# SHI-Labs/SH-GAN

Measured on AMD Instinct MI355X. Metric: generator images/sec, higher is better.
Workload: dtype f32

## Files before the change

include/shgan_hip.h:

```cpp
#ifndef SHGAN_HIP_H
#define SHGAN_HIP_H
#include <stddef.h>
#include <stdint.h>
#ifdef __cplusplus
extern "C" {
#endif

#define SHG_OK 0
#define SHG_ERR_ARG (-1)
#define SHG_ERR_LAUNCH (-2)
#define SHG_ERR_UNSUPPORTED (-3)

int shg_abi_version(void);
const char* shg_last_error(void);
int shg_device_info(int dev, char* buf, int buflen);

int shg_upfirdn2d_out_size(int H, int W, int fh, int fw, int upx, int upy, int downx, int downy, int padx0, int padx1,
                           int pady0, int pady1, int* OH, int* OW);
int shg_upfirdn2d_f32(const float* x, const float* f, float* y, int N, int C, int H, int W, int fh, int fw, int upx, int upy,
                      int downx, int downy, int padx0, int padx1, int pady0, int pady1, int flip, float gain, void* stream);
int shg_upfirdn2d_strided(const void* x, const float* f, void* y, int dtype, int N, int C, int H, int W, const long* x_strides,
                          const long* y_strides, int fh, int fw, long f_stride_y, long f_stride_x, int upx, int upy, int downx, int downy,
                          int padx0, int padx1, int pady0, int pady1, int flip, float gain, void* stream);
int shg_upfirdn2d_epilogue_f32(const float* x, const float* f, float* y, int N, int C, int H, int W, int fh, int fw, int upx,
// ... 54 lines not shown
                             int act, float alpha, float act_gain, float clamp, const float* residual, void* stream);
int shg_conv_weight_prep_up_poly_f32(const float* w, const float* wscale, float* wu_a, float* wu_b, int O, int I, int OP, int flip,
                                     void* stream);
int shg_conv2d_up_poly_supported(int NB, int I, int O, int H, int W);
int shg_conv2d_up_poly_f32(const float* x, const float* wt, const float* wu_a, const float* wu_b, float* y, int NB, int I, int O,
                           int OP, int H, int W, const float* in_scale, void* stream);
size_t shg_conv2d_up_poly_workspace_bytes(int NB, int I, int O, int OP, int H, int W);
int shg_conv2d_up_poly_ws_f32(const float* x, const float* wt, const float* wu_a, const float* wu_b, float* y, int NB, int I, int O,
                              int OP, int H, int W, const float* in_scale, void* workspace, size_t ws_bytes, void* stream);
int shg_fir_down_planar_f32(const float* x, const float* f, float* y, int N, int C, int H, int W, int PP, int flip, float gain,
                            void* stream);
int shg_fir_pad2_sep_supported(int H, int W, int PP);
int shg_fir_pad2_sep_f32(const float* x, const float* taps_host, float* y, int N, int C, int H, int W, int PP, int flip, float gain,
                         void* stream);
int shg_fir_resample2_sep_supported(int H, int W, int up);
int shg_fir_resample2_sep_f32(const float* x, const float* taps_host, float* y, int N, int C, int H, int W, int up, int flip, float gain,
                              void* stream);
int shg_conv_weight_prep_down_poly_f32(const float* w, const float* wscale, float* wu_a, float* wu_b, int O, int I, int OP, int flip,
                                       void* stream);
int shg_conv2d_down_poly_supported(int NB, int I, int O, int OH, int OW);
int shg_conv2d_down_poly_f32(const float* xp, const float* wu_a, const float* wu_b, float* y, int NB, int I, int O, int OP, int OH,
                             int OW, int PP, const float* in_scale, const float* bias, int act, float alpha, float gain,
                             float clamp, const float* residual, void* stream);
int shg_conv1x1_thin_in_f32(const float* x, const float* w, const float* bias, float* y, int N, int I, int O, int HW, float wgain,
                            int act, float alpha, float gain, float clamp, void* stream);
int shg_torgb_f32(const float* x, const float* w, const float* styles, const float* bias, const float* base_up, const float* f,
                  float* y, int N, int I, int O, int H, int W, void* stream);

int shg_dense_f32(const float* x, const float* w, const float* b, float* y, int N, int K, int O, int ldx, int ldy, float wgain,
                  float bgain, int act, float alpha, float gain, float clamp, void* stream);
int shg_matmul_nn_f32(const float* a, const float* b, float* out, int N, int M, int K, int lda, int ldo, float scale, void* stream);
int shg_matmul_tn_f32(const float* a, const float* b, float* out, float* colsum, int N, int M, int K, int lda, int ldb, float scale,
                      float csum_scale, void* stream);
int shg_demod_weight_f32(const float* w, float* wn, float* wsq, float* sfac, int O, int I, int K, int prenorm, void* stream);
int shg_demod_weight_backward_f32(const float* wn, const float* sfac, const float* gwn, const float* gwsq, float* gw, int O, int I, int K,
                                  void* stream);
int shg_style_factors_f32(const float* s, const float* wsq, float* sn, float* d, float* aux, int N, int I, int O, int prenorm, void* stream);
int shg_style_factors_backward_f32(const float* sn, const float* d, const float* wsq, const float* aux, const float* gsn, const float* gd,
                                   float* gs, float* gwsq, float* partq, int N, int I, int O, int prenorm, void* stream);
int shg_normalize_2nd_moment_f32(const float* x, float* y, int N, int K, float eps, void* stream);
int shg_modconv_style_prep_f32(const float* styles, int ld, const float* wsq, float* s_out, float* dcoef, int N, int I, int O,
                               int OP, int demod, float pre_gain, void* stream);

typedef struct {
    const float* x1; const float* x2; const float* w; const float* b; float* y;
    int ld1, ld2, K1, K2, O, ldy;
// ... 78 lines not shown
```

sh-gan_amd/_lib.py:

```python
import ctypes
import os

import torch

_HERE = os.path.dirname(os.path.abspath(__file__))
LIB_PATH = os.path.join(_HERE, 'lib', 'libshgan_hip.so')
ABI_VERSION = 38

c_fp = ctypes.c_void_p
c_i = ctypes.c_int
c_f = ctypes.c_float
c_l = ctypes.c_long
c_pp = ctypes.POINTER(ctypes.c_void_p)



class DenseGroup(ctypes.Structure):
    _fields_ = [('x1', c_fp), ('x2', c_fp), ('w', c_fp), ('b', c_fp), ('y', c_fp),
                ('ld1', c_i), ('ld2', c_i), ('K1', c_i), ('K2', c_i), ('O', c_i), ('ldy', c_i),
                ('wgain', c_f), ('bgain', c_f)]


class StyleGroup(ctypes.Structure):
    _fields_ = [('styles', c_fp), ('wsq', c_fp), ('s_out', c_fp), ('dcoef', c_fp),
                ('ld', c_i), ('I', c_i), ('O', c_i), ('OP', c_i), ('demod', c_i), ('pre_gain', c_f)]


_SIGS = {
    'shg_abi_version': [],
    'shg_device_info': [c_i, ctypes.c_char_p, c_i],
# ... 47 lines not shown
    'shg_conv2d_wgrad_f32': [c_fp, c_fp, c_fp] + [c_i] * 11 + [c_fp, ctypes.c_size_t, c_fp],
    'shg_conv2d_wgrad_wino_supported': [c_i] * 8,
    'shg_conv2d_wgrad_wino_workspace_bytes': [c_i] * 5,
    'shg_conv2d_wgrad_wino_f32': [c_fp, c_fp, c_fp] + [c_i] * 5 + [c_fp, ctypes.c_size_t, c_fp],
    'shg_shu_spectral_f32': [c_fp] * 6 + [c_i] * 4 + [c_fp],
    'shg_shu_split_irfft2_f32': [c_fp, c_fp, c_pp, c_pp, ctypes.POINTER(c_l), c_i, c_i, c_i, c_i, c_fp],
    'shg_shu_split_adjoint_f32': [c_pp, ctypes.POINTER(c_l), c_pp, c_fp, c_i, c_i, c_fp],
    'shg_composite_u8': [c_fp, c_fp, c_fp, c_i, c_i, c_i, c_fp],
    'shg_assemble_input_f32': [c_fp, c_fp, c_fp, c_i, c_i, c_i, c_fp],
    'shg_assemble_input_u8': [c_fp, c_fp, c_fp, c_fp, c_i, c_i, c_i, c_fp],
    'shg_conv_weight_prep_up_poly_f32': [c_fp, c_fp, c_fp, c_fp, c_i, c_i, c_i, c_i, c_fp],
    'shg_conv2d_up_poly_supported': [c_i, c_i, c_i, c_i, c_i],
    'shg_conv2d_up_poly_f32': [c_fp, c_fp, c_fp, c_fp, c_fp, c_i, c_i, c_i, c_i, c_i, c_i, c_fp, c_fp],
    'shg_conv2d_up_poly_ws_f32': [c_fp, c_fp, c_fp, c_fp, c_fp] + [c_i] * 6 + [c_fp, c_fp, ctypes.c_size_t, c_fp],
    'shg_conv2d_up_poly_workspace_bytes': [c_i] * 6,
    'shg_fir_down_planar_f32': [c_fp, c_fp, c_fp, c_i, c_i, c_i, c_i, c_i, c_i, c_f, c_fp],
    'shg_fir_pad2_sep_supported': [c_i, c_i, c_i],
    'shg_fir_resample2_sep_supported': [c_i, c_i, c_i],
    'shg_fir_resample2_sep_f32': [c_fp, ctypes.POINTER(c_f), c_fp, c_i, c_i, c_i, c_i, c_i, c_i, c_f, c_fp],
    'shg_fir_pad2_sep_f32': [c_fp, ctypes.POINTER(c_f), c_fp, c_i, c_i, c_i, c_i, c_i, c_i, c_f, c_fp],
    'shg_conv_weight_prep_down_poly_f32': [c_fp, c_fp, c_fp, c_fp, c_i, c_i, c_i, c_i, c_fp],
    'shg_conv2d_down_poly_supported': [c_i, c_i, c_i, c_i, c_i],
    'shg_conv2d_down_poly_f32': [c_fp, c_fp, c_fp, c_fp, c_i, c_i, c_i, c_i, c_i, c_i, c_i, c_fp, c_fp, c_i, c_f, c_f, c_f, c_fp, c_fp],
    'shg_mask_raster_f32': [c_fp, c_fp, c_fp, c_fp, c_i, c_fp, c_fp, c_i, c_i, c_fp],
    'shg_fid_accumulate_f64': [c_fp, c_i, c_fp, c_fp, c_i, c_i, c_i, c_fp],
    'shg_image_metrics_scratch_bytes': [c_i] * 4,
    'shg_image_metrics': [c_fp, c_fp, c_f, c_f, c_fp, c_fp, c_f, c_f] + [c_i] * 6 + [c_fp, ctypes.c_size_t, c_fp, c_fp, c_fp],
    'shg_resize_bicubic_u8': [c_fp, c_l, c_fp, c_l, c_fp, c_i, c_i, c_i, c_i, c_i, c_fp],
    'shg_minibatch_std_f32': [c_fp, c_fp, c_fp, c_i, c_i, c_i, c_i, c_i, c_i, c_fp],
    'shg_conv2d_f16': [c_fp, c_fp, c_fp, c_fp] + [c_i] * 12 + [c_fp],
    'shg_conv2d_f16_needs_clear': [c_i] * 5,
    'shg_conv2d_f16_fused': [c_fp, c_fp, c_fp] + [c_i] * 12 + [c_fp, c_fp, c_fp, c_i, c_f, c_fp, c_i, c_f, c_f, c_f, c_fp, c_fp],
    'shg_conv2d_f16_packed_weight_elems': [c_i] * 3,
    'shg_conv2d_f16_pack_weight': [c_fp, c_fp, c_i, c_i, c_i, c_fp],
    'shg_conv2d_f16_pack_weight_oihw': [c_fp, c_fp, c_i, c_i, c_i, c_i, c_i, c_fp],
    'shg_conv2d_f16_set_routes': [c_i],
    'shg_conv2d_wgrad_f16_workspace_bytes': [c_i] * 6,
    'shg_conv2d_wgrad_f16': [c_fp, c_fp, c_fp] + [c_i] * 10 + [c_fp, ctypes.c_size_t, c_fp],
    'shg_upfirdn2d_f16': [c_fp, c_fp, c_fp] + [c_i] * 15 + [c_f, c_fp],
    'shg_relayout_f32_f16': [c_fp, c_fp, c_i, c_i, c_l, c_i, c_fp],
    'shg_bias_act_f16': [c_fp, c_fp, c_fp, c_l, c_i, c_i, c_f, c_f, c_f, c_fp],
    'shg_bias_act_backward_f16': [c_fp, c_fp, c_fp, c_l, c_i, c_f, c_f, c_f, c_fp],
    'shg_modtail_backward_f32_blocks': [c_l],
    'shg_modtail_backward_f32_cslices': [c_i, c_i, c_l],
    'shg_modtail_backward_f32': [c_fp] * 9 + [c_i, c_i, c_l, c_i, c_f, c_f, c_f, c_fp],
    'shg_modtail_f16': [c_fp, c_fp, c_fp, c_i, c_fp, c_fp, c_i, c_l, c_i, c_i, c_f, c_f, c_f, c_fp],
# ... 18 lines not shown
    if _lib is not None:
        return _lib
    if not os.path.exists(LIB_PATH):
        raise RuntimeError(
            f'{LIB_PATH} not found: the HIP extension is not built. Run `python sh-gan_amd/build.py` '
            '(or __graft_entry__.build()). There is deliberately no CPU / PyTorch fallback.')
    lib = ctypes.CDLL(LIB_PATH)
    for name, args in _SIGS.items():
        fn = getattr(lib, name)
        fn.argtypes = args
        fn.restype = c_i
    lib.shg_last_error.argtypes = []
    lib.shg_last_error.restype = ctypes.c_char_p
    lib.shg_conv2d_workspace_bytes.restype = ctypes.c_size_t
    lib.shg_conv2d_wgrad_workspace_bytes.restype = ctypes.c_size_t
    lib.shg_conv2d_wino_workspace_bytes.restype = ctypes.c_size_t
    lib.shg_conv2d_wino4_workspace_bytes.restype = ctypes.c_size_t
    lib.shg_conv2d_up_poly_workspace_bytes.restype = ctypes.c_size_t
    lib.shg_conv2d_wgrad_wino_workspace_bytes.restype = ctypes.c_size_t
    lib.shg_conv2d_wgrad_f16_workspace_bytes.restype = ctypes.c_size_t
    lib.shg_image_metrics_scratch_bytes.restype = ctypes.c_size_t
    lib.shg_conv2d_f16_packed_weight_elems.restype = c_l
    lib.shg_conv_wino4_weight_elems.restype = c_l
    ver = lib.shg_abi_version()
    if ver != ABI_VERSION:
        raise RuntimeError(f'libshgan_hip.so ABI {ver} != expected {ABI_VERSION}: rebuild with sh-gan_amd/build.py')
    _lib = lib
    return lib


def exported_symbols():
    return sorted(list(_SIGS.keys()) + ['shg_last_error'])


def check(rc, what=''):
    if rc != 0:
        msg = get_lib().shg_last_error().decode(errors='replace')
        raise ShgError(f'{what}: {msg} (code {rc})')
```

sh-gan_amd/build.py:

```python
import hashlib
import os
import subprocess
import sys

HERE = os.path.dirname(os.path.abspath(__file__))
CSRC = os.path.join(HERE, 'csrc')
LIBDIR = os.path.join(HERE, 'lib')
LIBNAME = 'libshgan_hip.so'
VARDIR = os.path.join(os.path.dirname(HERE), 'tools', '_variants')
SOURCES = ['capi.hip', 'upfirdn2d.hip', 'pointwise.hip', 'dense.hip', 'conv_mfma.hip', 'conv_wino.hip', 'conv_wino4.hip', 'conv_wino_poly.hip', 'conv_wgrad.hip', 'conv_wgrad_wino.hip', 'conv_f16.hip', 'conv_f16_ring.hip', 'conv_f16_upring.hip', 'conv_f16_down.hip', 'shu.hip', 'mask_raster.hip', 'fid_stats.hip', 'image_metrics.hip', 'resize.hip']
SRC_FLAGS = {'conv_wgrad_wino.hip': ['-fno-slp-vectorize']}
FLAGS = ['--offload-arch=gfx950', '-O3', '-std=c++17', '-fPIC', '-fno-gpu-rdc', '-Wall', '-Wno-unused-function', '-Wno-inline-asm']


def _hipcc():
    for c in (os.environ.get('HIPCC'), '/opt/rocm/bin/hipcc', 'hipcc'):
        if c and (os.path.isabs(c) and os.path.exists(c) or not os.path.isabs(c)):
            return c
    raise RuntimeError('hipcc not found')


INCLUDE = os.path.join(os.path.dirname(HERE), 'include')


def _digest(extra=()):
    h = hashlib.sha256()
    for d in (CSRC, INCLUDE):
        for name in sorted(os.listdir(d)):
            with open(os.path.join(d, name), 'rb') as fh:
                h.update(name.encode())
                h.update(fh.read())
    h.update(' '.join(list(FLAGS) + [f'{k}:{v}' for k, v in sorted(SRC_FLAGS.items())] + list(extra)).encode())
    return h.hexdigest()
# ... 54 lines not shown
```

sh-gan_amd/csrc/capi.hip:

```cpp
#include "shg_common.h"
#include <string.h>

static thread_local char g_err[512] = "";

void shg_set_error(const char* fmt, ...) {
    va_list ap;
    va_start(ap, fmt);
    vsnprintf(g_err, sizeof(g_err), fmt, ap);
    va_end(ap);
}

extern "C" const char* shg_last_error(void) { return g_err; }

extern "C" int shg_abi_version(void) { return 38; }

extern "C" int shg_device_info(int dev, char* buf, int buflen) {
    hipDeviceProp_t prop;
    hipError_t e = hipGetDeviceProperties(&prop, dev);
    if (e != hipSuccess) {
        shg_set_error("hipGetDeviceProperties(%d): %s", dev, hipGetErrorString(e));
        return SHG_ERR_LAUNCH;
    }
    if (buf && buflen > 0) {
        strncpy(buf, prop.gcnArchName, buflen - 1);
        buf[buflen - 1] = 0;
    }
    return prop.multiProcessorCount;
}
```

sh-gan_amd/kernels.py:

```python
import contextlib
import ctypes
import math

import torch

from . import _lib
from ._lib import check

SQRT2 = math.sqrt(2.0)
_NULLCTX = contextlib.nullcontext()


class _Launch:
    __slots__ = ('dev', 'keep', '_ctx')

    def __init__(self):
        self.dev = None
        self.keep = []
        self._ctx = None

    def _own(self, t, name):
        if self.dev is None:
            self.dev = t.device
        elif t.device != self.dev:
# ... 465 lines not shown

def assemble_input(real, mask, lut=None):
    L = _Launch()
    u8 = isinstance(real, torch.Tensor) and real.dtype == torch.uint8
    real = L.req(real, 'real', dtype=torch.uint8 if u8 else torch.float32)
    mask = L.req(mask, 'mask')
    n, c, h, w = real.shape
    if c != 3 or mask.numel() != n * h * w:
        raise _lib.ShgError('assemble_input: real must be [N,3,H,W] and mask [N,(1,)H,W]')
    x = L.new((n, 4, h, w))
    with L:
        if u8:
            lut = L.req(u8_value_table(L.dev) if lut is None else lut, 'lut')
            if lut.numel() != 256:
                raise _lib.ShgError('assemble_input: lut must hold 256 floats')
            check(_lib.get_lib().shg_assemble_input_u8(_ptr(real), _ptr(mask), _ptr(lut), _ptr(x), n, h, w, L.stream()), 'assemble_input_u8')
        else:
            check(_lib.get_lib().shg_assemble_input_f32(_ptr(real), _ptr(mask), _ptr(x), n, h, w, L.stream()), 'assemble_input')
    return x



class PreppedWeight:
    __slots__ = ('wt', 'wsq', 'o', 'i', 'op', 'kh', 'kw', 'groups', 'wu', 'wu4', 'wu_up', 'wu_down', '_w', '_wscale', '_flip')

    def __init__(self, wt, wsq, o, i, op, kh, kw, groups=1, w=None, wscale=None, flip=False):
        self.wt, self.wsq, self.o, self.i, self.op, self.kh, self.kw, self.groups = wt, wsq, o, i, op, kh, kw, groups
        self.wu, self.wu4, self.wu_up, self.wu_down, self._w, self._wscale, self._flip = None, None, None, None, w, wscale, flip

    def _poly(self, entry):
        if self._w is None or self.groups != 1 or self.kh != 3 or self.kw != 3:
            raise _lib.ShgError('PreppedWeight: polyphase forms need an ungrouped 3x3 weight')
        L = _Launch()
        w, ws = L.req(self._w, 'w'), L.req(self._wscale, 'wscale')
        size = (self.op // 64) * ((self.i + 7) // 8) * 16 * 64 * 8
        wa, wb = L.new((size,)), L.new((size,))
        with L:
            check(getattr(_lib.get_lib(), entry)(_ptr(w), _ptr(ws), _ptr(wa), _ptr(wb), self.o, self.i, self.op,
                                                 int(bool(self._flip)), L.stream()), entry)
        return wa, wb

    def down_poly(self):
        if self.wu_down is None:
            self.wu_down = self._poly('shg_conv_weight_prep_down_poly_f32')
        return self.wu_down

    def up_poly(self):
        if self.wu_up is None:
            self.wu_up = self._poly('shg_conv_weight_prep_up_poly_f32')
        return self.wu_up

    def wino(self):
        if self.wu is None:
            if self._w is None or self.groups != 1 or self.kh != 3 or self.kw != 3:
                raise _lib.ShgError('PreppedWeight.wino: needs an ungrouped 3x3 weight')
            L = _Launch()
            w, ws = L.req(self._w, 'w'), L.req(self._wscale, 'wscale')
            kc = int(_lib.get_lib().shg_conv_wino_chunk())
            nchunk = (self.i + kc - 1) // kc
            self.wu = L.new(((self.op // 64) * nchunk * 16 * 64 * kc,))
            with L:
                check(_lib.get_lib().shg_conv_weight_prep_wino_f32(_ptr(w), _ptr(ws), _ptr(self.wu), self.o, self.i, self.op,
                                                                   int(bool(self._flip)), L.stream()), 'conv_weight_prep_wino')
        return self.wu

    def wino4(self):
        if self.wu4 is None:
            if self._w is None or self.groups != 1 or self.kh != 3 or self.kw != 3:
# ... 93 lines not shown
        nba, nbb = ((h + 1 + 2) // 3) * ((w + 1 + 2) // 3), (h // 2) * (w // 2)
        executed = 2.0 * nb * pw.o * i * (16.0 * (nba + nbb) + h + w)
        ws_bytes = int(lib.shg_conv2d_up_poly_workspace_bytes(nb, i, pw.o, pw.op, h, w)) if WINO_SPLIT else 0
        ws = L.new((ws_bytes // 4,)) if ws_bytes else None
        with _timed(L, 'conv_poly_up', 2.0 * nb * pw.o * i * 9 * h * w, executed):
            check(lib.shg_conv2d_up_poly_ws_f32(_ptr(x), _ptr(pw.wt), _ptr(wa), _ptr(wb), _ptr(y), nb, i, pw.o, pw.op, h, w,
                                                _ptr(in_scale), _ptr(ws), ws_bytes, L.stream()), 'conv2d_up_poly')
        return y
    ws, ws_bytes = None, 0
    if mode != MODE_UP2T or planar:
        ws_bytes = int(lib.shg_conv2d_workspace_bytes(nb, i, pw.o, h, w, pw.kh, pw.kw, mode, pad, pw.groups))
        if ws_bytes:
            ws = L.new((ws_bytes // 4,))
    pix = (h * w) if mode == MODE_UP2T else (oh * ow)
    with _timed(L, _CONV_CLASS[mode] if pw.kh == 3 else 'conv_mfma_1x1', 2.0 * nb * pw.o * i * pw.kh * pw.kw * pix):
        check(lib.shg_conv2d_f32(
            _ptr(x), _ptr(pw.wt), _ptr(y), nb, i, pw.o, pw.op, h, w, pw.kh, pw.kw, mode, pad, pw.groups, pw.wt.shape[1],
            _ptr(in_scale), _ptr(out_scale), _ptr(bias), _ptr(noise), nmode, float(noise_strength), a, al, g, cl, _ptr(residual),
            1 if planar else 0, _ptr(ws), ws_bytes, L.stream()), 'conv2d')
    return y


DOWN_POLY_MIN_I, DOWN_POLY_MIN_OUT = 128, 32


def down_poly_supported(x, pw, force=False):
    n, i, h, w = x.shape
    if not force and (i < DOWN_POLY_MIN_I or min(h, w) // 2 < DOWN_POLY_MIN_OUT):
        return False
    return bool(DOWN_POLY and pw.groups == 1 and pw.kh == 3 and pw.kw == 3 and pw._w is not None and h % 2 == 0 and w % 2 == 0
                and x.is_cuda and _lib.get_lib().shg_conv2d_down_poly_supported(n, i, pw.o, h // 2, w // 2))


def fir_conv_down2(x, f, pw, bias=None, act=False, gain=1.0, alpha=0.2, act_gain=SQRT2, clamp=256.0, residual=None, flip_filter=False):
    L = _Launch()
    x, f = L.req(x, 'x'), L.req(f, 'f')
    if tuple(f.shape) != (4, 4):
        raise _lib.ShgError('fir_conv_down2: f must be 4x4')
    n, i, h, w = x.shape
    oh, ow = h // 2, w // 2
    lib = _lib.get_lib()
    pp4 = (ow + 1 + 3) // 4 * 4
    taps = sep_taps(f) if lib.shg_fir_pad2_sep_supported(h, w, pp4) else None
    pp = (ow + 1 + 31) // 32 * 32 if (taps is not None and w % 256 == 0) else pp4
    wa, wb = pw.down_poly()
    L.view(wa, 'weights')
    xp = L.new((4, n, i, oh + 1, pp))
    y = L.new((n, pw.o, oh, ow))
    bias, residual = L.req(bias, 'bias'), L.req(residual, 'residual')
    if residual is not None and tuple(residual.shape) != tuple(y.shape):
        raise _lib.ShgError('fir_conv_down2: residual shape mismatch')
    a, al, g, cl = _act_args(act, gain, alpha, act_gain, clamp)
    with _timed(L, 'upfirdn2d', 4.0 * (x.numel() + n * i * (h + 1) * (w + 1))):
        if taps is not None:
            check(lib.shg_fir_pad2_sep_f32(_ptr(x), taps, _ptr(xp), n, i, h, w, pp, int(bool(flip_filter)), 1.0, L.stream()), 'fir_pad2_sep')
        else:
            check(lib.shg_fir_down_planar_f32(_ptr(x), _ptr(f), _ptr(xp), n, i, h, w, pp, int(bool(flip_filter)), 1.0, L.stream()),
                  'fir_down_planar')
    nba, nbb = ((oh + 2) // 3) * ((ow + 2) // 3), (oh // 2) * (ow // 2)
    with _timed(L, 'conv_poly_down', 2.0 * n * pw.o * i * 9 * oh * ow, 2.0 * n * pw.o * i * 16.0 * (nba + nbb)):
        check(lib.shg_conv2d_down_poly_f32(_ptr(xp), _ptr(wa), _ptr(wb), _ptr(y), n, i, pw.o, pw.op, oh, ow, pp, None, _ptr(bias),
                                           a, al, g, cl, _ptr(residual), L.stream()), 'conv2d_down_poly')
    return y


def upfir_planar(mid, f, scale=None, bias=None, noise=None, noise_strength=1.0, residual=None, act=False, gain=1.0,
                 alpha=0.2, act_gain=SQRT2, clamp=256.0, fir_gain=4.0, flip=False):
    L = _Launch()
    mid = L.req(mid, 'mid')
    f = L.req(f, 'f')
    if mid.ndim != 5 or mid.shape[0] != 4 or tuple(f.shape) != (4, 4):
        raise _lib.ShgError('upfir_planar: mid must be [4,N,C,H+1,W+1] and f 4x4')
    _, n, c, hp, wp = mid.shape
    h, w = hp - 1, wp - 1
    y = L.new((n, c, 2 * h, 2 * w))
    noise, nmode = _noise_args(L, noise, n)
    a, al, g, cl = _act_args(act, gain, alpha, act_gain, clamp)
    residual = L.req(residual, 'residual')
    scale, bias = L.req(scale, 'scale'), L.req(bias, 'bias')
    if residual is not None and tuple(residual.shape) != tuple(y.shape):
        raise _lib.ShgError('upfir_planar: residual shape mismatch')
# ... 336 lines not shown
```

Measured before the change: 820.8.

## Add stacked-polyphase Winograd F(4,2) kernel for low-channel stride-2 downsample convs

Adds a new MFMA kernel that treats the four polyphase planes of a stride-2 3x3 conv as one stacked 2x2 conv over 4*I channels. It runs that conv with a Winograd F(4x4,2x2) transform, using 25 positions per 4x4 output block. Input transforms run on dedicated waves that overlap with MFMA waves, and raw tiles are fetched by async LDS DMA into double buffers. The route is used for layers with I<=64, which the old poly kernel path skipped because of its channel minimum. The change adds a new weight-prep cache and some FP32 Winograd numerical error.

```diff
diff --git a/include/shgan_hip.h b/include/shgan_hip.h
--- a/include/shgan_hip.h
+++ b/include/shgan_hip.h
@@ -100,6 +100,11 @@
 int shg_conv2d_down_poly_f32(const float* xp, const float* wu_a, const float* wu_b, float* y, int NB, int I, int O, int OP, int OH,
                              int OW, int PP, const float* in_scale, const float* bias, int act, float alpha, float gain,
                              float clamp, const float* residual, void* stream);
+long shg_conv_down_stack_weight_elems(int OP, int I);
+int shg_conv_weight_prep_down_stack_f32(const float* w, const float* wscale, float* wu, int O, int I, int OP, int flip, void* stream);
+int shg_conv2d_down_stack_supported(int NB, int I, int O, int OH, int OW);
+int shg_conv2d_down_stack_f32(const float* xp, const float* wu, float* y, int NB, int I, int O, int OP, int OH, int OW, int PP,
+                              const float* bias, int act, float alpha, float gain, float clamp, const float* residual, void* stream);
 int shg_conv1x1_thin_in_f32(const float* x, const float* w, const float* bias, float* y, int N, int I, int O, int HW, float wgain,
                             int act, float alpha, float gain, float clamp, void* stream);
 int shg_torgb_f32(const float* x, const float* w, const float* styles, const float* bias, const float* base_up, const float* f,
diff --git a/sh-gan_amd/_lib.py b/sh-gan_amd/_lib.py
--- a/sh-gan_amd/_lib.py
+++ b/sh-gan_amd/_lib.py
@@ -5,7 +5,7 @@
 
 _HERE = os.path.dirname(os.path.abspath(__file__))
 LIB_PATH = os.path.join(_HERE, 'lib', 'libshgan_hip.so')
-ABI_VERSION = 38
+ABI_VERSION = 39
 
 c_fp = ctypes.c_void_p
 c_i = ctypes.c_int
@@ -99,6 +99,10 @@
     'shg_conv_weight_prep_down_poly_f32': [c_fp, c_fp, c_fp, c_fp, c_i, c_i, c_i, c_i, c_fp],
     'shg_conv2d_down_poly_supported': [c_i, c_i, c_i, c_i, c_i],
     'shg_conv2d_down_poly_f32': [c_fp, c_fp, c_fp, c_fp, c_i, c_i, c_i, c_i, c_i, c_i, c_i, c_fp, c_fp, c_i, c_f, c_f, c_f, c_fp, c_fp],
+    'shg_conv_down_stack_weight_elems': [c_i, c_i],
+    'shg_conv_weight_prep_down_stack_f32': [c_fp, c_fp, c_fp, c_i, c_i, c_i, c_i, c_fp],
+    'shg_conv2d_down_stack_supported': [c_i, c_i, c_i, c_i, c_i],
+    'shg_conv2d_down_stack_f32': [c_fp, c_fp, c_fp] + [c_i] * 7 + [c_fp, c_i, c_f, c_f, c_f, c_fp, c_fp],
     'shg_mask_raster_f32': [c_fp, c_fp, c_fp, c_fp, c_i, c_fp, c_fp, c_i, c_i, c_fp],
     'shg_fid_accumulate_f64': [c_fp, c_i, c_fp, c_fp, c_i, c_i, c_i, c_fp],
     'shg_image_metrics_scratch_bytes': [c_i] * 4,
@@ -163,6 +167,7 @@
     lib.shg_image_metrics_scratch_bytes.restype = ctypes.c_size_t
     lib.shg_conv2d_f16_packed_weight_elems.restype = c_l
     lib.shg_conv_wino4_weight_elems.restype = c_l
+    lib.shg_conv_down_stack_weight_elems.restype = c_l
     ver = lib.shg_abi_version()
     if ver != ABI_VERSION:
         raise RuntimeError(f'libshgan_hip.so ABI {ver} != expected {ABI_VERSION}: rebuild with sh-gan_amd/build.py')
diff --git a/sh-gan_amd/build.py b/sh-gan_amd/build.py
--- a/sh-gan_amd/build.py
+++ b/sh-gan_amd/build.py
@@ -8,7 +8,7 @@
 LIBDIR = os.path.join(HERE, 'lib')
 LIBNAME = 'libshgan_hip.so'
 VARDIR = os.path.join(os.path.dirname(HERE), 'tools', '_variants')
-SOURCES = ['capi.hip', 'upfirdn2d.hip', 'pointwise.hip', 'dense.hip', 'conv_mfma.hip', 'conv_wino.hip', 'conv_wino4.hip', 'conv_wino_poly.hip', 'conv_wgrad.hip', 'conv_wgrad_wino.hip', 'conv_f16.hip', 'conv_f16_ring.hip', 'conv_f16_upring.hip', 'conv_f16_down.hip', 'shu.hip', 'mask_raster.hip', 'fid_stats.hip', 'image_metrics.hip', 'resize.hip']
+SOURCES = ['capi.hip', 'upfirdn2d.hip', 'pointwise.hip', 'dense.hip', 'conv_mfma.hip', 'conv_wino.hip', 'conv_wino4.hip', 'conv_wino_poly.hip', 'conv_down_stack.hip', 'conv_wgrad.hip', 'conv_wgrad_wino.hip', 'conv_f16.hip', 'conv_f16_ring.hip', 'conv_f16_upring.hip', 'conv_f16_down.hip', 'shu.hip', 'mask_raster.hip', 'fid_stats.hip', 'image_metrics.hip', 'resize.hip']
 SRC_FLAGS = {'conv_wgrad_wino.hip': ['-fno-slp-vectorize']}
 FLAGS = ['--offload-arch=gfx950', '-O3', '-std=c++17', '-fPIC', '-fno-gpu-rdc', '-Wall', '-Wno-unused-function', '-Wno-inline-asm']
 
diff --git a/sh-gan_amd/csrc/capi.hip b/sh-gan_amd/csrc/capi.hip
--- a/sh-gan_amd/csrc/capi.hip
+++ b/sh-gan_amd/csrc/capi.hip
@@ -12,7 +12,7 @@
 
 extern "C" const char* shg_last_error(void) { return g_err; }
 
-extern "C" int shg_abi_version(void) { return 38; }
+extern "C" int shg_abi_version(void) { return 39; }
 
 extern "C" int shg_device_info(int dev, char* buf, int buflen) {
     hipDeviceProp_t prop;
diff --git a/sh-gan_amd/csrc/conv_down_stack.hip b/sh-gan_amd/csrc/conv_down_stack.hip
--- /dev/null
+++ b/sh-gan_amd/csrc/conv_down_stack.hip
@@ -0,0 +1,403 @@
+#include "shg_common.h"
+#include <stdlib.h>
+#include <type_traits>
+
+typedef float f32x16 __attribute__((ext_vector_type(16)));
+typedef float f32x4 __attribute__((ext_vector_type(4)));
+
+__device__ __attribute__((aligned(16))) float shg_dstack_zeros[64];
+
+struct DStackParams {
+    const float* xp;
+    const float* wu;
+    float* y;
+    const float* bias;
+    const float* residual;
+    int NB, I, O, OP, OH, OW, PH2, PP;
+    int tiles_x, tiles_y, n_ttiles, n_otiles, nchunk;
+    int act;
+    float alpha, gain, clamp;
+};
+
+namespace dstack {
+constexpr int KC = 8, BO = 64, BT = 32, NPOS = 25, NW = 8, NT = NW * 64, NUNIT = 2 * NPOS;
+constexpr int V_SZ = NPOS * KC * BT;
+template <int TY, int TX>
+struct Tile {
+    static_assert(TY * TX == BT, "32 blocks per tile");
+    static constexpr int PH = 4 * TY + 1, PW = 4 * TX + 4, PW4 = PW / 4, PATCH4 = PH * PW4;
+    static constexpr int NPIECE = (PATCH4 + 63) / 64, RP = NPIECE * 256, R_SZ = KC * RP;
+    static_assert(NPIECE <= 3, "a fetch wave issues its 2 * NPIECE window pieces behind its first six MFMAs");
+};
+static_assert(2 * V_SZ >= NPOS * 16 * 32, "epilogue exchange buffer lives in the V region");
+__host__ __device__ constexpr int unit_first(int w) { return w < 4 ? 6 * w : (w == 4 ? 24 : (w == 5 ? 30 : (w == 6 ? 37 : 43))); }
+}
+
+__device__ __forceinline__ int dstack_xcd_remap(int bid, int total) {
+    const int q = total >> 3, r = total & 7;
+    const int xcd = bid & 7, idx = bid >> 3;
+    const int base = xcd < r ? xcd * (q + 1) : r * (q + 1) + (xcd - r) * q;
+    return base + idx;
+}
+
+__device__ __forceinline__ void dstack_bt(const float (&d)[5], float (&o)[5]) {
+    const float e = d[3] - d[1];
+    o[0] = 2.f * (d[0] - d[2]) + e;
+    o[1] = 2.f * d[1] + d[2] - d[3];
+    o[2] = 3.f * d[2] - 2.f * d[1] - d[3];
+    o[3] = e;
+    o[4] = 2.f * (d[1] - d[3]) - d[2] + d[4];
+}
+__device__ __forceinline__ void dstack_at(const float (&m)[5], float (&o)[4]) {
+    const float s12 = m[1] + m[2], d12 = m[1] - m[2];
+    o[0] = m[0] + s12 + m[3];
+    o[1] = d12 + 2.f * m[3];
+    o[2] = s12 + 4.f * m[3];
+    o[3] = d12 + 8.f * m[3] + m[4];
+}
+
+template <int TY, int TX>
+__global__ __launch_bounds__(512, 2) void conv_down_stack_kernel(const DStackParams p) {
+    using namespace dstack;
+    using T = Tile<TY, TX>;
+    constexpr int PW = T::PW, PW4 = T::PW4, PATCH4 = T::PATCH4, RP = T::RP, R_SZ = T::R_SZ, NPIECE = T::NPIECE;
+    __shared__ __attribute__((aligned(16))) float Vl[2 * V_SZ];
+    __shared__ __attribute__((aligned(16))) float Rl[2 * R_SZ];
+
+    const int tid = threadIdx.x;
+    const int lane = tid & 63, wave = __builtin_amdgcn_readfirstlane(tid >> 6);
+    const int l31 = lane & 31, half = lane >> 5;
+
+    const int nwork = p.n_ttiles * p.n_otiles;
+    const int work = dstack_xcd_remap(blockIdx.x, nwork);
+    const int otile = work / p.n_ttiles;
+    const int ttile = work - otile * p.n_ttiles;
+    const int txb = ttile % p.tiles_x;
+    const int tyb = (ttile / p.tiles_x) % p.tiles_y;
+    const int n = ttile / (p.tiles_x * p.tiles_y);
+    const int oy0 = tyb * (4 * TY), ox0 = txb * (4 * TX);
+    const int o0 = otile * BO;
+    const int HW = p.PH2 * p.PP;
+    const int nch = p.nchunk, K4 = 4 * p.I;
+
+    const bool xformer = wave < 4;
+    int roff[NPIECE];
+#pragma unroll
+    for (int j = 0; j < NPIECE; ++j) {
+        const int q = j * 64 + lane;
+        const int py = q / PW4, p4 = q - py * PW4;
+        const int iy = oy0 + py, ix = ox0 + 4 * p4;
+        const bool ok = q < PATCH4 && iy < p.PH2 && ix + 3 < p.PP;
+        roff[j] = ok ? iy * p.PP + ix : -1;
+    }
+    auto dma_piece = [&](int c, int buf, int q, int j) __attribute__((always_inline)) {
+        const int k = (wave - 4) * 2 + q;
+        const int ch = c * KC + k;
+        const int ab = ch / p.I, i = ch - ab * p.I;
+        const float* src = (ch < K4 && roff[j] >= 0) ? p.xp + ((long)((ab * p.NB + n) * p.I + i) * HW + roff[j]) : shg_dstack_zeros;
+        const unsigned lds = __builtin_amdgcn_readfirstlane(
+            (unsigned)(size_t)(__attribute__((address_space(3))) void*)(Rl + buf * R_SZ + k * RP + j * 256));
+        asm volatile("s_mov_b32 m0, %0\n\ts_nop 0\n\tglobal_load_lds_dwordx4 %1, off" ::"s"(lds), "v"(src) : "m0", "memory");
+    };
+    auto dma_raw = [&](int c, int buf) __attribute__((always_inline)) {
+#pragma unroll
+        for (int q = 0; q < 2; ++q)
+#pragma unroll
+            for (int j = 0; j < NPIECE; ++j) dma_piece(c, buf, q, j);
+    };
+
+    const int tty = l31 / TX, ttx = l31 % TX;
+    const float* rbase = Rl + (2 * wave + half) * RP + (4 * tty) * PW + 4 * ttx;
+    float* vbase = Vl + (2 * wave + half) * BT + l31;
+    auto tr_read = [&](int r, f32x4& w4, float& w1, int buf) __attribute__((always_inline)) {
+        const float* rb = rbase + buf * R_SZ + r * PW;
+        w4 = *reinterpret_cast<const f32x4*>(rb);
+        w1 = rb[4];
+    };
+    auto tr_row = [&](int r, const f32x4& w4, float w1, float (&u)[5][5]) __attribute__((always_inline)) {
+        const float di[5] = {w4[0], w4[1], w4[2], w4[3], w1};
+        dstack_bt(di, u[r]);
+    };
+    auto tr_col = [&](int j, const float (&u)[5][5], int buf) __attribute__((always_inline)) {
+        float* vb = vbase + buf * V_SZ + j * KC * BT;
+        const float di[5] = {u[0][j], u[1][j], u[2][j], u[3][j], u[4][j]};
+        float o[5];
+        dstack_bt(di, o);
+#pragma unroll
+        for (int i = 0; i < 5; ++i) vb[i * 5 * KC * BT] = o[i];
+    };
+
+    float* Mx = Vl;
+    const long plane = (long)p.OH * p.OW;
+    const int o_l = tid >> 5, t_l = tid & 31;
+    const int by = t_l / TX, bx = t_l % TX;
+    const int oy = oy0 + 4 * by, ox = ox0 + 4 * bx;
+
+    auto body = [&](auto nu_c, auto xf_c) __attribute__((always_inline)) {
+        constexpr int NU = decltype(nu_c)::value;
+        constexpr bool XF = decltype(xf_c)::value;
+        const int ufirst = unit_first(wave);
+        constexpr size_t ustride = (size_t)4 * NUNIT * 64;
+        const float* ubase = p.wu + ((size_t)otile * p.nchunk * 4 * NUNIT + ufirst) * 64 + lane;
+        float ur[4][NU];
+        auto load_u = [&](int c, int ks) __attribute__((always_inline)) {
+#pragma unroll
+            for (int j = 0; j < NU; ++j) ur[ks][j] = ubase[(size_t)c * ustride + (ks * NUNIT + j) * 64];
+        };
+        f32x16 acc[NU];
+#pragma unroll
+        for (int j = 0; j < NU; ++j)
+#pragma unroll
+            for (int r = 0; r < 16; ++r) acc[j][r] = 0.f;
+        const float* bbase = Vl + half * BT + l31;
+        int boff[NU];
+#pragma unroll
+        for (int j = 0; j < NU; ++j) boff[j] = ((ufirst + j) >> 1) * KC * BT;
+
+        float b[2][NU];
+#pragma unroll
+        for (int ks = 0; ks < 3; ++ks) load_u(0, ks);
+#pragma unroll
+        for (int j = 0; j < NU; ++j) ur[3][j] = 0.f;
+#pragma unroll
+        for (int q = 0; q < NU; ++q) b[1][q] = 0.f;
+        if constexpr (!XF) {
+            dma_raw(0, 0);
+            dma_raw(1, 1);
+        }
+        __builtin_amdgcn_s_waitcnt(0x0F70);
+        __syncthreads();
+        if constexpr (XF) {
+            f32x4 w4;
+            float w1, u[5][5];
+#pragma unroll
+            for (int r = 0; r < 5; ++r) {
+                tr_read(r, w4, w1, 0);
+                tr_row(r, w4, w1, u);
+            }
+#pragma unroll
+            for (int j = 0; j < 5; ++j) tr_col(j, u, 0);
+        }
+        __syncthreads();
+
+        const int last = nch - 1;
+        auto fetch = [&](const float* bb, int ks, int pb) __attribute__((always_inline)) {
+#pragma unroll
+            for (int q = 0; q < NU; ++q) b[pb][q] = bb[boff[q] + ks * 2 * BT];
+        };
+        auto mma = [&](int ks, int pb, int j) __attribute__((always_inline)) {
+            acc[j] = __builtin_amdgcn_mfma_f32_32x32x2f32(ur[ks][j], b[pb][j], acc[j], 0, 0, 0);
+        };
+        auto refill = [&](int c, int ks, int j) __attribute__((always_inline)) {
+            ur[ks][j] = ubase[(size_t)c * ustride + (ks * NUNIT + j) * 64];
+        };
+        for (int c = 0; c < nch; ++c) {
+            const int buf = c & 1;
+            const int cn = c < last ? c + 1 : last;
+            const float* bb = bbase + buf * V_SZ;
+            f32x4 w4[2];
+            float w1[2];
+            float u[5][5];
+            fetch(bb, 0, 0);
+            __builtin_amdgcn_sched_barrier(0);
+            constexpr int RFD = 2;
+            auto refill_m = [&](int m) __attribute__((always_inline)) {
+                if (m / NU == 0) refill(c, 3, m % NU);
+                else refill(cn, m / NU - 1, m % NU);
+            };
+#pragma unroll
+            for (int j = 0; j < NU; ++j) {
+                mma(3, 1, j);
+                if constexpr (!XF) {
+                    if (j < 2 * NPIECE) dma_piece(c + 2, buf, j / NPIECE, j % NPIECE);
+                }
+                if (j >= RFD) refill_m(j - RFD);
+                if constexpr (XF) {
+                    if (j < 5) tr_read(j, w4[j & 1], w1[j & 1], buf ^ 1);
+                    if (j >= 1 && j < 6) tr_row(j - 1, w4[(j - 1) & 1], w1[(j - 1) & 1], u);
+                }
+                __builtin_amdgcn_sched_barrier(0);
+            }
+#pragma unroll
+            for (int ks = 0; ks < 3; ++ks) {
+                fetch(bb, ks + 1, (ks + 1) & 1);
+                __builtin_amdgcn_sched_barrier(0);
+#pragma unroll
+                for (int j = 0; j < NU; ++j) {
+                    mma(ks, ks & 1, j);
+                    refill_m((ks + 1) * NU + j - RFD);
+                    if constexpr (XF) {
+                        if (ks == 0 && j < 5) tr_col(j, u, buf ^ 1);
+                    }
+                    __builtin_amdgcn_sched_barrier(0);
+                }
+            }
+#pragma unroll
+            for (int m = 4 * NU - RFD; m < 4 * NU; ++m) refill_m(m);
+            if constexpr (!XF) asm volatile("s_waitcnt vmcnt(%0)" ::"n"(4 * NU - 2 * NPIECE + 1 + RFD) : "memory");
+            asm volatile("s_waitcnt lgkmcnt(0)" ::: "memory");
+            __builtin_amdgcn_s_barrier();
+            asm volatile("" ::: "memory");
+        }
+#pragma unroll
+        for (int j = 0; j < NU; ++j) mma(3, 1, j);
+
+        const bool col_ok = oy < p.OH && ox < p.OW;
+        const int oxc = ox < p.OW ? ox : 0;
+        long rowoff[4];
+#pragma unroll
+        for (int i = 0; i < 4; ++i) rowoff[i] = (long)(oy + i < p.OH ? oy + i : p.OH - 1) * p.OW + oxc;
+        struct TailOps { float bs; f32x4 rs[4]; };
+        auto tail_load = [&](int pass, TailOps& t) __attribute__((always_inline)) {
+            const int oo = o0 + (pass >> 1) * 32 + 16 * (pass & 1) + o_l;
+            const int oc = oo < p.O ? oo : p.O - 1;
+            t.bs = p.bias ? p.bias[oc] : 0.f;
+            const float* rp = p.residual ? p.residual + ((long)n * p.O + oc) * plane : shg_dstack_zeros;
+#pragma unroll
+            for (int i = 0; i < 4; ++i) t.rs[i] = *reinterpret_cast<const f32x4*>(rp + (p.residual ? rowoff[i] : 0));
+        };
+        auto finish = [&](int pass, TailOps& t) __attribute__((always_inline)) {
+            const int ob = pass >> 1, h = pass & 1;
+            const int o = o0 + ob * 32 + 16 * h + o_l;
+            float tmp[5][4];
+#pragma unroll
+            for (int r = 0; r < 5; ++r) {
+                float m[5], a4[4];
+#pragma unroll
+                for (int cc = 0; cc < 5; ++cc) m[cc] = Mx[((r * 5 + cc) * 16 + o_l) * 32 + t_l];
+                dstack_at(m, a4);
+#pragma unroll
+                for (int k = 0; k < 4; ++k) tmp[r][k] = a4[k];
+            }
+            f32x4 out[4];
+#pragma unroll
+            for (int k = 0; k < 4; ++k) {
+                const float col[5] = {tmp[0][k], tmp[1][k], tmp[2][k], tmp[3][k], tmp[4][k]};
+                float a4[4];
+                dstack_at(col, a4);
+#pragma unroll
+                for (int i = 0; i < 4; ++i) {
+                    float v = a4[i] + t.bs;
+                    v = p.act ? shg_lrelu_agc(v, p.alpha, p.gain, p.clamp) : v * p.gain;
+                    out[i][k] = v + t.rs[i][k];
+                }
+            }
+            if (pass < 3) tail_load(pass + 1, t);
+            if (o < p.O && col_ok) {
+                float* yp = p.y + ((long)n * p.O + o) * plane;
+#pragma unroll
+                for (int i = 0; i < 4; ++i)
+                    if (oy + i < p.OH) *reinterpret_cast<f32x4*>(yp + rowoff[i]) = out[i];
+            }
+        };
+
+        TailOps tops;
+        tail_load(0, tops);
+#pragma unroll
+        for (int pass = 0; pass < 4; ++pass) {
+            const int ob = pass >> 1, h = pass & 1;
+#pragma unroll
+            for (int j = 0; j < NU; ++j) {
+                const int unit = ufirst + j;
+                if ((unit & 1) != ob) continue;
+#pragma unroll
+                for (int rr = 0; rr < 8; ++rr) {
+                    const int r = 8 * h + rr;
+                    const int lr = (r & 3) + 8 * ((r >> 2) & 1) + 4 * half;
+                    Mx[((unit >> 1) * 16 + lr) * 32 + l31] = acc[j][r];
+                }
+            }
+            __syncthreads();
+            finish(pass, tops);
+            if (pass < 3) __syncthreads();
+        }
+    };
+    if (xformer) body(std::integral_constant<int, 6>{}, std::true_type{});
+    else if (wave == 4 || wave == 6) body(std::integral_constant<int, 6>{}, std::false_type{});
+    else body(std::integral_constant<int, 7>{}, std::false_type{});
+}
+
+__global__ __launch_bounds__(256) void dstack_weight_kernel(const float* w, const float* scale, float* wu, int O, int I, int OP,
+                                                            int nchunk, int flip) {
+    constexpr int KC = dstack::KC;
+    const long e = (long)blockIdx.x * 256 + threadIdx.x;
+    const long total = (long)OP * nchunk * KC;
+    if (e >= total) return;
+    const int o = (int)(e % OP);
+    const int k = (int)(e / OP);
+    const int ab = k / I, i = k - ab * I, a = ab >> 1, b = ab & 1;
+    float g[2][2];
+#pragma unroll
+    for (int dy = 0; dy < 2; ++dy)
+#pragma unroll
+        for (int dx = 0; dx < 2; ++dx) {
+            const int ky = 2 * dy + a, kx = 2 * dx + b;
+            const int t = ky * 3 + kx, tt = flip ? 8 - t : t;
+            g[dy][dx] = (o < O && ab < 4 && ky <= 2 && kx <= 2) ? w[((long)o * I + i) * 9 + tt] * scale[o] : 0.f;
+        }
+    auto gcol = [](float g0, float g1, float (&r)[5]) {
+        r[0] = 0.5f * g0;
+        r[1] = 0.5f * (g0 + g1);
+        r[2] = (g0 - g1) * (1.f / 6.f);
+        r[3] = g0 * (1.f / 6.f) + g1 * (1.f / 3.f);
+        r[4] = g1;
+    };
+    float c0[5], c1[5];
+    gcol(g[0][0], g[1][0], c0);
+    gcol(g[0][1], g[1][1], c1);
+    const int kc = k % KC, chunk = k / KC;
+    const int ln = (kc & 1) * 32 + (o & 31), ks = kc >> 1, obk = (o & 63) >> 5;
+    float* base = wu + ((size_t)(o >> 6) * nchunk + chunk) * (4 * dstack::NUNIT * 64);
+#pragma unroll
+    for (int r = 0; r < 5; ++r) {
+        float row[5];
+        gcol(c0[r], c1[r], row);
+#pragma unroll
+        for (int cc = 0; cc < 5; ++cc) base[((size_t)ks * dstack::NUNIT + (r * 5 + cc) * 2 + obk) * 64 + ln] = row[cc];
+    }
+}
+
+extern "C" long shg_conv_down_stack_weight_elems(int OP, int I) {
+    return (long)(OP / 64) * shg_cdiv(4L * I, dstack::KC) * 4 * dstack::NUNIT * 64;
+}
+
+extern "C" int shg_conv_weight_prep_down_stack_f32(const float* w, const float* wscale, float* wu, int O, int I, int OP, int flip,
+                                                   void* stream) {
+    SHG_CHECK_ARG(w && wscale && wu, "weight_prep_down_stack: null pointer");
+    SHG_CHECK_ARG(O >= 1 && I >= 1 && OP % 64 == 0 && OP >= O, "weight_prep_down_stack: bad shape");
+    const int nchunk = shg_cdiv(4L * I, dstack::KC);
+    const long total = (long)OP * nchunk * dstack::KC;
+    hipLaunchKernelGGL(dstack_weight_kernel, dim3(shg_cdiv(total, 256)), dim3(256), 0, (hipStream_t)stream, w, wscale, wu, O, I, OP,
+                       nchunk, flip);
+    SHG_CHECK_LAUNCH();
+    return SHG_OK;
+}
+
+extern "C" int shg_conv2d_down_stack_supported(int NB, int I, int O, int OH, int OW) {
+    return (OH >= 4 && OW >= 16 && OW % 4 == 0 && I >= 1 && I <= 1024 && NB >= 1 && O >= 1) ? 1 : 0;
+}
+
+extern "C" int shg_conv2d_down_stack_f32(const float* xp, const float* wu, float* y, int NB, int I, int O, int OP, int OH, int OW, int PP,
+                                         const float* bias, int act, float alpha, float gain, float clamp, const float* residual,
+                                         void* stream) {
+    SHG_CHECK_ARG(xp && wu && y, "conv2d_down_stack: null pointer");
+    SHG_CHECK_ARG(shg_conv2d_down_stack_supported(NB, I, O, OH, OW), "conv2d_down_stack: unsupported geometry");
+    SHG_CHECK_ARG(OP % 64 == 0 && OP >= O, "conv2d_down_stack: OP must be a multiple of 64 and >= O");
+    SHG_CHECK_ARG(PP % 4 == 0 && PP >= OW + 1, "conv2d_down_stack: plane pitch must be a multiple of 4 and >= OW + 1");
+    SHG_CHECK_ARG(4L * NB * I * (OH + 1) * PP < 2147483647L && (long)NB * O * OH * OW < 2147483647L, "conv2d_down_stack: tensor too large");
+    SHG_CHECK_ARG(((reinterpret_cast<uintptr_t>(xp) | reinterpret_cast<uintptr_t>(y) | reinterpret_cast<uintptr_t>(residual)) & 15) == 0,
+                  "conv2d_down_stack: xp / y / residual must be 16-byte aligned");
+    DStackParams p{};
+    p.xp = xp; p.wu = wu; p.y = y; p.bias = bias; p.residual = residual;
+    p.NB = NB; p.I = I; p.O = O; p.OP = OP; p.OH = OH; p.OW = OW; p.PH2 = OH + 1; p.PP = PP;
+    p.act = act; p.alpha = alpha; p.gain = gain; p.clamp = clamp;
+    const int shape = (OW >= 256) ? 2 : (OW >= 128 ? 1 : 0);
+    p.tiles_x = shg_cdiv(OW, 32 << shape); p.tiles_y = shg_cdiv(OH, 16 >> shape);
+    p.n_ttiles = p.tiles_x * p.tiles_y * NB; p.n_otiles = OP / 64; p.nchunk = shg_cdiv(4L * I, dstack::KC);
+    const dim3 grid(p.n_ttiles * p.n_otiles);
+    if (shape == 2) hipLaunchKernelGGL((conv_down_stack_kernel<1, 32>), grid, dim3(dstack::NT), 0, (hipStream_t)stream, p);
+    else if (shape == 1) hipLaunchKernelGGL((conv_down_stack_kernel<2, 16>), grid, dim3(dstack::NT), 0, (hipStream_t)stream, p);
+    else hipLaunchKernelGGL((conv_down_stack_kernel<4, 8>), grid, dim3(dstack::NT), 0, (hipStream_t)stream, p);
+    SHG_CHECK_LAUNCH();
+    return SHG_OK;
+}
diff --git a/sh-gan_amd/kernels.py b/sh-gan_amd/kernels.py
--- a/sh-gan_amd/kernels.py
+++ b/sh-gan_amd/kernels.py
@@ -511,11 +511,12 @@
 
 
 class PreppedWeight:
-    __slots__ = ('wt', 'wsq', 'o', 'i', 'op', 'kh', 'kw', 'groups', 'wu', 'wu4', 'wu_up', 'wu_down', '_w', '_wscale', '_flip')
+    __slots__ = ('wt', 'wsq', 'o', 'i', 'op', 'kh', 'kw', 'groups', 'wu', 'wu4', 'wu_up', 'wu_down', 'wu_dstack', '_w', '_wscale', '_flip')
 
     def __init__(self, wt, wsq, o, i, op, kh, kw, groups=1, w=None, wscale=None, flip=False):
         self.wt, self.wsq, self.o, self.i, self.op, self.kh, self.kw, self.groups = wt, wsq, o, i, op, kh, kw, groups
         self.wu, self.wu4, self.wu_up, self.wu_down, self._w, self._wscale, self._flip = None, None, None, None, w, wscale, flip
+        self.wu_dstack = None
 
     def _poly(self, entry):
         if self._w is None or self.groups != 1 or self.kh != 3 or self.kw != 3:
@@ -533,6 +534,20 @@
         if self.wu_down is None:
             self.wu_down = self._poly('shg_conv_weight_prep_down_poly_f32')
         return self.wu_down
+
+    def down_stack(self):
+        if self.wu_dstack is None:
+            if self._w is None or self.groups != 1 or self.kh != 3 or self.kw != 3:
+                raise _lib.ShgError('PreppedWeight: polyphase forms need an ungrouped 3x3 weight')
+            lib = _lib.get_lib()
+            L = _Launch()
+            w, ws = L.req(self._w, 'w'), L.req(self._wscale, 'wscale')
+            wu = L.new((int(lib.shg_conv_down_stack_weight_elems(self.op, self.i)),))
+            with L:
+                check(lib.shg_conv_weight_prep_down_stack_f32(_ptr(w), _ptr(ws), _ptr(wu), self.o, self.i, self.op,
+                                                              int(bool(self._flip)), L.stream()), 'weight_prep_down_stack')
+            self.wu_dstack = wu
+        return self.wu_dstack
 
     def up_poly(self):
         if self.wu_up is None:
@@ -672,14 +687,29 @@
 
 
 DOWN_POLY_MIN_I, DOWN_POLY_MIN_OUT = 128, 32
+DOWN_STACK = True
+DOWN_STACK_MAX_I = 64
+
+
+def _down_route(x, pw):
+    n, i, h, w = x.shape
+    if not (DOWN_POLY and pw.groups == 1 and pw.kh == 3 and pw.kw == 3 and pw._w is not None and h % 2 == 0 and w % 2 == 0
+            and x.is_cuda):
+        return None
+    lib = _lib.get_lib()
+    if DOWN_STACK and i <= DOWN_STACK_MAX_I and lib.shg_conv2d_down_stack_supported(n, i, pw.o, h // 2, w // 2):
+        return 'stack'
+    if lib.shg_conv2d_down_poly_supported(n, i, pw.o, h // 2, w // 2):
+        return 'poly'
+    return None
 
 
 def down_poly_supported(x, pw, force=False):
     n, i, h, w = x.shape
-    if not force and (i < DOWN_POLY_MIN_I or min(h, w) // 2 < DOWN_POLY_MIN_OUT):
+    if not force and min(h, w) // 2 < DOWN_POLY_MIN_OUT:
         return False
-    return bool(DOWN_POLY and pw.groups == 1 and pw.kh == 3 and pw.kw == 3 and pw._w is not None and h % 2 == 0 and w % 2 == 0
-                and x.is_cuda and _lib.get_lib().shg_conv2d_down_poly_supported(n, i, pw.o, h // 2, w // 2))
+    route = _down_route(x, pw)
+    return route is not None and (force or route == 'stack' or i >= DOWN_POLY_MIN_I)
 
 
 def fir_conv_down2(x, f, pw, bias=None, act=False, gain=1.0, alpha=0.2, act_gain=SQRT2, clamp=256.0, residual=None, flip_filter=False):
@@ -693,7 +723,8 @@
     pp4 = (ow + 1 + 3) // 4 * 4
     taps = sep_taps(f) if lib.shg_fir_pad2_sep_supported(h, w, pp4) else None
     pp = (ow + 1 + 31) // 32 * 32 if (taps is not None and w % 256 == 0) else pp4
-    wa, wb = pw.down_poly()
+    stack = _down_route(x, pw) == 'stack'
+    wa, wb = (pw.down_stack(), None) if stack else pw.down_poly()
     L.view(wa, 'weights')
     xp = L.new((4, n, i, oh + 1, pp))
     y = L.new((n, pw.o, oh, ow))
@@ -707,6 +738,12 @@
         else:
             check(lib.shg_fir_down_planar_f32(_ptr(x), _ptr(f), _ptr(xp), n, i, h, w, pp, int(bool(flip_filter)), 1.0, L.stream()),
                   'fir_down_planar')
+    if stack:
+        nb4 = ((oh + 3) // 4) * ((ow + 3) // 4)
+        with _timed(L, 'conv_poly_down', 2.0 * n * pw.o * i * 9 * oh * ow, 2.0 * n * pw.o * 4 * i * 25.0 * nb4):
+            check(lib.shg_conv2d_down_stack_f32(_ptr(xp), _ptr(wa), _ptr(y), n, i, pw.o, pw.op, oh, ow, pp, _ptr(bias),
+                                                a, al, g, cl, _ptr(residual), L.stream()), 'conv2d_down_stack')
+        return y
     nba, nbb = ((oh + 2) // 3) * ((ow + 2) // 3), (oh // 2) * (ow // 2)
     with _timed(L, 'conv_poly_down', 2.0 * n * pw.o * i * 9 * oh * ow, 2.0 * n * pw.o * i * 16.0 * (nba + nbb)):
         check(lib.shg_conv2d_down_poly_f32(_ptr(xp), _ptr(wa), _ptr(wb), _ptr(y), n, i, pw.o, pw.op, oh, ow, pp, None, _ptr(bias),
diff --git a/sh-gan_amd/wino_down_ref.py b/sh-gan_amd/wino_down_ref.py
--- /dev/null
+++ b/sh-gan_amd/wino_down_ref.py
@@ -0,0 +1,105 @@
+import numpy as np
+from fractions import Fraction as Fr
+
+POINTS = {
+    3: [0, 1, -1, 'inf'],
+    4: [0, 1, -1, 2, 'inf'],
+    6: [0, 1, -1, 2, -2, Fr(1, 2), 'inf'],
+}
+
+
+def _mat_inv(m):
+    n = len(m)
+    a = [list(r) + [Fr(int(i == j)) for j in range(n)] for i, r in enumerate(m)]
+    for c in range(n):
+        p = next(r for r in range(c, n) if a[r][c] != 0)
+        a[c], a[p] = a[p], a[c]
+        pv = a[c][c]
+        a[c] = [v / pv for v in a[c]]
+        for r in range(n):
+            if r != c and a[r][c] != 0:
+                f = a[r][c]
+                a[r] = [vr - f * vc for vr, vc in zip(a[r], a[c])]
+    return [r[n:] for r in a]
+
+
+def transforms(m, points=None):
+    pts = [Fr(p) if p != 'inf' else p for p in (points or POINTS[m])]
+    n = m + 1
+    assert len(pts) == n
+    def ev(deg):
+        return [[(p ** k if p != 'inf' else Fr(int(k == deg - 1))) for k in range(deg)] for p in pts]
+    V = ev(n)
+    Vinv = _mat_inv(V)
+    BT = [[Vinv[j][i] for j in range(n)] for i in range(n)]
+    G = ev(2)
+    AT = [[r[i] for r in ev(m)] for i in range(m)]
+    for j in range(n):
+        den = 1
+        for v in BT[j]:
+            den = den * v.denominator // np.gcd(den, v.denominator)
+        if den != 1:
+            BT[j] = [v * den for v in BT[j]]
+            G[j] = [v / den for v in G[j]]
+    f = lambda M: np.array([[float(v) for v in r] for r in M], dtype=np.float64)
+    return f(AT), f(G), f(BT)
+
+
+def stack_weights(w):
+    O, I = w.shape[:2]
+    w2 = np.zeros((O, 4, I, 2, 2), w.dtype)
+    for a in range(2):
+        for b in range(2):
+            for dy in range(2):
+                for dx in range(2):
+                    ky, kx = 2 * dy + a, 2 * dx + b
+                    if ky <= 2 and kx <= 2:
+                        w2[:, 2 * a + b, :, dy, dx] = w[:, :, ky, kx]
+    return w2.reshape(O, 4 * I, 2, 2)
+
+
+def polyphase(xf, oh, ow):
+    out = np.zeros((xf.shape[0], 4 * xf.shape[1], oh + 1, ow + 1), xf.dtype)
+    for a in range(2):
+        for b in range(2):
+            pl = xf[:, :, a::2, b::2][:, :, :oh + 1, :ow + 1]
+            out[:, (2 * a + b) * xf.shape[1]:(2 * a + b + 1) * xf.shape[1], :pl.shape[2], :pl.shape[3]] = pl
+    return out
+
+
+def conv_stack_emulated(ps, w2, m, dtype=np.float32):
+    AT, G, BT = (t.astype(dtype) for t in transforms(m))
+    n_ = m + 1
+    N, K, PH, PW = ps.shape
+    O = w2.shape[0]
+    oh, ow = PH - 1, PW - 1
+    nby, nbx = -(-oh // m), -(-ow // m)
+    pad = np.zeros((N, K, nby * m + 1, nbx * m + 1), dtype)
+    pad[:, :, :PH, :PW] = ps
+    U = np.einsum('ac,okcd,bd->abok', G, w2.astype(dtype), G).astype(dtype)
+    d = np.lib.stride_tricks.sliding_window_view(pad, (n_, n_), axis=(2, 3))[:, :, ::m, ::m].astype(dtype)
+    V = np.einsum('ai,nkyxij,bj->abknyx', BT, d, BT).astype(dtype)
+    M = np.einsum('abok,abknyx->abonyx', U, V).astype(dtype)
+    Y = np.einsum('ia,abonyx,jb->nyixjo', AT, M, AT).astype(dtype)
+    Y = Y.reshape(N, nby * m, nbx * m, O).transpose(0, 3, 1, 2)
+    return Y[:, :, :oh, :ow]
+
+
+def conv_stack_reference(ps, w2):
+    ps, w2 = ps.astype(np.float64), w2.astype(np.float64)
+    oh, ow = ps.shape[2] - 1, ps.shape[3] - 1
+    y = 0
+    for dy in range(2):
+        for dx in range(2):
+            y = y + np.einsum('ok,nkyx->noyx', w2[:, :, dy, dx], ps[:, :, dy:dy + oh, dx:dx + ow])
+    return y
+
+
+def error_of(m, n, ci, co, oh, ow, seed=0):
+    rs = np.random.RandomState(seed)
+    ps = rs.standard_normal((n, 4 * ci, oh + 1, ow + 1)).astype(np.float32)
+    w = (rs.standard_normal((co, ci, 3, 3)) * 0.05).astype(np.float32)
+    w2 = stack_weights(w)
+    y = conv_stack_emulated(ps, w2, m)
+    r = conv_stack_reference(ps, w2)
+    return float(np.abs(y - r).max() / np.abs(r).max())
```

Result: no change. 826.1, median of 6 (+0.7%).
